# CMU-SAFARI/Genome-on-Diet

Hardware: AMD Instinct MI355X
Metric: mapped bases/sec (whole node), HiFi map-hifi k19w19 (higher is better)
Workload: dtype int16

## Files before the change

### genome-on-diet_amd/csrc/ksw_wave.hip.h

```cpp
#pragma once
#include <hip/hip_runtime.h>
#include <type_traits>
#include "ksw_common.h"
#include "ksw_wave_core.h"

template <int LANES> __device__ __forceinline__ u32 gdw_ror1(u32 v)
{
	if (LANES != 16) return (u32)__builtin_amdgcn_mov_dpp((int)v, 0x13C, 0xF, 0xF, true);
	return (u32)__builtin_amdgcn_mov_dpp((int)v, 0x121, 0xF, 0xF, true);
}

__device__ __forceinline__ u32 gdw_seam_byte(const uint8_t *query, int qlen, int j)
{
	if (j < 0 || j >= qlen) return 0u;
	const uintptr_t a = (uintptr_t)(query + j);
	typedef const __attribute__((address_space(4))) u32 *gdw_const_u32p;
	const u32 wd = *(gdw_const_u32p)(a & ~(uintptr_t)3);
	return (wd >> (8 * (a & 3))) & 0xffu;
}

__device__ __forceinline__ void gdw_band_uniform(int r, int qlen, int tlen, int w, int &st0, int &en0)
{
	r = __builtin_amdgcn_readfirstlane(r);
	int a = r - qlen + 1, b = (r - w + 1) >> 1, c = (r + w) >> 1, t1 = tlen - 1, st, en;
// ... 3 lines not shown
}

__device__ __forceinline__ const uint8_t *gdw_uniform_ptr(const uint8_t *p, int src_lane)
{
	const uintptr_t a = (uintptr_t)p;
	const u32 lo = (u32)__builtin_amdgcn_readlane((int)(u32)a, src_lane), hi = (u32)__builtin_amdgcn_readlane((int)(u32)(a >> 32), src_lane);
	return (const uint8_t *)((uintptr_t)hi << 32 | lo);
}
__device__ __forceinline__ int64_t gdw_uniform_i64(int64_t v)
{
	const u32 lo = (u32)__builtin_amdgcn_readfirstlane((int)(u32)(uint64_t)v), hi = (u32)__builtin_amdgcn_readfirstlane((int)(u32)((uint64_t)v >> 32));
	return (int64_t)((uint64_t)hi << 32 | lo);
}

#if __has_builtin(__builtin_amdgcn_writelane)
#define GDW_WRITELANE __builtin_amdgcn_writelane
#else
extern "C" __device__ int gdw_llvm_writelane_i32(int, int, int) __asm("llvm.amdgcn.writelane.i32");
#define GDW_WRITELANE gdw_llvm_writelane_i32
#endif
__device__ __forceinline__ u32 gdw_writelane_u(u32 value_uniform, int lane_uniform, u32 old)
{
	return (u32)GDW_WRITELANE(__builtin_amdgcn_readfirstlane((int)value_uniform), __builtin_amdgcn_readfirstlane(lane_uniform), (int)old);
}

__device__ __forceinline__ int gdw_narrow_rows(const WaveK &K, const uint8_t *query_u , const uint8_t *query, int qlen,
                                               const uint8_t *target, int tlen, int w, int lane, __amdgpu_buffer_rsrc_t bt_rsrc)
{
	typedef u32 gdw_u32x2 __attribute__((ext_vector_type(2)));
	const int rend = qlen + tlen - 2, mlast = (tlen - 1) >> 4, sl = (tlen - 1) & 15;
	WaveHalf H;
	gdw_load_half(H, K, lane >> 1, lane & 1, 0, query, qlen, target, tlen);
	bool any_tn = __builtin_amdgcn_ballot_w64(H.tn != 0) != 0;
	int prev_st_ = 0, prev_st0 = -1, prev_up = -1, prev_en0 = -1, have_f = 0, Rf = 0;
	auto store_row = [&](const int r, const u32 out[2]) __attribute__((always_inline)) {
		const gdw_u32x2 d = {out[0], out[1]};
		__builtin_amdgcn_raw_buffer_store_b64(d, bt_rsrc, lane * 8, r * 512, 0);
	};
	auto dp_row = [&](const int r, auto steady_tag) __attribute__((always_inline)) {
		constexpr bool STEADY = decltype(steady_tag)::value;
		WaveRow W;
		W.r = r;
		gdw_band_uniform(r, qlen, tlen, w, W.st0, W.en0);
		W.st_ = W.st0 >> 4, W.en_ = W.en0 >> 4;
		W.up = W.st0 + (((W.en0 - W.st0 + 16) >> 4) << 4);
		const int advanced = W.st_ > prev_st_;
		W.use_array = advanced;
		W.v1key = STEADY ? K.key_open : (W.st_ == 0 ? gdw_edge_key(K, r) : K.key_open);
		W.set_tr = STEADY ? 0 : (W.en0 | 15) >= r;
		W.ukey = STEADY ? 0 : gdw_edge_key(K, r);
		const u32 pX = gdw_ror1<64>(H.X[3]), pV = gdw_ror1<64>(H.V[3]), pX2 = gdw_ror1<64>(H.X2[3]), pQ = gdw_ror1<64>(H.Qc[1]);
		if (STEADY || r > 0) gdw_shift_query_half(H, pQ, H.blk == prev_st_ && H.half == 0, gdw_seam_byte(query_u, qlen, r - (prev_st_ << 4)));
		if (advanced) {
			if (H.blk < W.st_) gdw_load_half(H, K, H.blk + 32, H.half, r, query, qlen, target, tlen);
			any_tn = __builtin_amdgcn_ballot_w64(H.tn != 0) != 0;
		}
		if (!STEADY && W.set_tr) gdw_reset_tr_half(H, K, W);
		if (W.st0 != prev_st0 || W.up != prev_up || advanced) gdw_make_sel_half(H, W.st0, W.up);
		gdw_update_scores_half(H, K, any_tn);
		if (H.blk <= W.en_) {
			u32 out[2];
			gdw_compute_half<true>(H, K, W, pX, pV, pX2, out);
			store_row(r, out);
		}
		if (!STEADY && r == 0) H.R = gdw_lo(H.V[0]) - K.B1 - K.qe8;
		else H.R += gdw_lo(H.V[0]) - K.B1;
		if ((STEADY || r > 0) && W.en0 != prev_en0 && (W.en0 & 7) == 0) {
			const int hh = (int)gdw_ror1<64>((u32)gdw_track_handoff_half(H));
			if (H.blk == W.en_ && H.half == ((W.en0 >> 3) & 1)) H.R = hh + gdw_lo(H.U[0]);
		}
		if (!STEADY && W.en0 == tlen - 1) {
			if (H.blk == mlast && H.half == (sl >> 3)) {
				if (!have_f) Rf = gdw_track_to_slot_half(H, sl & 7);
				else Rf += gdw_cell_half(H.V, sl & 7) - K.B1;
			}
			have_f = 1;
		}
		prev_st_ = W.st_, prev_st0 = W.st0, prev_up = W.up, prev_en0 = W.en0;
	};
	const int nblkA = (w - 1 + 16) >> 4, nblkB = (w + 16) >> 4;
	u32 m_lowest = 0;
	const int step_mask = nblkA == nblkB ? 15 : 0;
	int m_full = 0;
	auto pair_row = [&](const int r, const int m, auto a_tag) __attribute__((always_inline)) {
		constexpr bool ROW_A = decltype(a_tag)::value;
		WaveRow W;
		W.r = r, W.st0 = m, W.en0 = ROW_A ? m + w - 1 : m + w;
		W.st_ = m >> 4, W.en_ = W.en0 >> 4;
		W.up = m + ((ROW_A ? nblkA : nblkB) << 4);
		const int advanced = ROW_A && (m & 15) == 0;
		const int pst_ = (m - (ROW_A ? 1 : 0)) >> 4;
		W.use_array = advanced, W.v1key = K.key_open, W.set_tr = 0, W.ukey = 0;
		const u32 pX = gdw_ror1<64>(H.X[3]), pV = gdw_ror1<64>(H.V[3]), pX2 = gdw_ror1<64>(H.X2[3]), pQ = gdw_ror1<64>(H.Qc[1]);
		gdw_shift_query_half_m(H, pQ, m_lowest, gdw_seam_byte(query_u, qlen, r - (pst_ << 4)));
		if (advanced) {
			if (H.blk < W.st_) gdw_load_half(H, K, H.blk + 32, H.half, r, query, qlen, target, tlen);
			any_tn = __builtin_amdgcn_ballot_w64(H.tn != 0) != 0;
		}
		if (ROW_A ? (m & step_mask) == 0 || m == m_full : nblkA != nblkB) {
			gdw_make_sel_half(H, W.st0, W.up);
			m_lowest = (H.blk == W.st_ && H.half == 0) ? ~0u : 0u;
		} else if (ROW_A) {
			const GdwSelStep S = gdw_sel_step_half(m, w);
#pragma unroll
			for (int k = 0; k < 2; ++k)
#pragma unroll
				for (int g = 0; g < 2; ++g) H.SEL[g] = gdw_writelane_u(S.sel[k][g], S.lane[k], H.SEL[g]);
		}
		W.m_first_valid = 1, W.m_first_h = m_lowest;
		gdw_update_scores_half(H, K, any_tn);
		if (H.blk <= W.en_) {
			u32 out[2];
			gdw_compute_half<true>(H, K, W, pX, pV, pX2, out);
			store_row(r, out);
		}
		H.R += gdw_lo(H.V[0]);
		if (!ROW_A && (W.en0 & 7) == 0) {
			const int hh = (int)gdw_ror1<64>((u32)gdw_track_handoff_half(H));
			if (H.blk == W.en_ && H.half == ((W.en0 >> 3) & 1)) H.R = hh + gdw_lo(H.U[0]);
		}
	};
	{
		int rA, rS;
		gdw_steady_rows(qlen, tlen, w, rA, rS);
		const int t1_ = tlen - 1, rB0 = 2 * t1_ - w, rB = rB0 > t1_ ? rB0 : t1_;
		int r = 0;
		for (; r <= rend && r < rA; ++r) dp_row(r, std::false_type());
		if (r == rA && rS > rA) {
			int m = (rA - w + 1) >> 1;
			m_full = m;
			m_lowest = (H.blk == prev_st_ && H.half == 0) ? ~0u : 0u;
			for (; r < rS; r += 2, ++m) {
				pair_row(r, m, std::true_type());
				pair_row(r + 1, m, std::false_type());
			}
			H.R -= (rS - rA) * K.B1;
			--m;
			prev_st_ = m >> 4, prev_st0 = m, prev_up = m + (nblkB << 4), prev_en0 = m + w;
		}
		for (; r <= rend && r < rB; ++r) dp_row(r, std::true_type());
		for (; r <= rend; ++r) dp_row(r, std::false_type());
	}
	return __builtin_amdgcn_readlane(Rf, (2 * mlast + (sl >> 3)) & 63);
}

__device__ __forceinline__ int gdw_quarter_rows(const WaveK &K, const uint8_t *query_u , const uint8_t *query, int qlen,
                                               const uint8_t *target, int tlen, int w, int lane, __amdgpu_buffer_rsrc_t bt_rsrc)
{
	const int rend = qlen + tlen - 2, mlast = (tlen - 1) >> 4, sl = (tlen - 1) & 15;
	WaveQuarter H;
	gdw_load_quarter(H, K, lane >> 2, lane & 3, 0, query, qlen, target, tlen);
	bool any_tn = __builtin_amdgcn_ballot_w64(H.tn != 0) != 0;
	int prev_st_ = 0, prev_st0 = -1, prev_up = -1, prev_en0 = -1, have_f = 0, Rf = 0;
	auto store_row = [&](const int r, const u32 out) __attribute__((always_inline)) {
		__builtin_amdgcn_raw_buffer_store_b32(out, bt_rsrc, lane * 4, r * 256, 0);
	};
	auto dp_row = [&](const int r, auto steady_tag) __attribute__((always_inline)) {
		constexpr bool STEADY = decltype(steady_tag)::value;
		WaveRow W;
		W.r = r;
		gdw_band_uniform(r, qlen, tlen, w, W.st0, W.en0);
		W.st_ = W.st0 >> 4, W.en_ = W.en0 >> 4;
		W.up = W.st0 + (((W.en0 - W.st0 + 16) >> 4) << 4);
		const int advanced = W.st_ > prev_st_;
		W.use_array = advanced;
		W.v1key = STEADY ? K.key_open : (W.st_ == 0 ? gdw_edge_key(K, r) : K.key_open);
		W.set_tr = STEADY ? 0 : (W.en0 | 15) >= r;
		W.ukey = STEADY ? 0 : gdw_edge_key(K, r);
		const u32 pX = gdw_ror1<64>(H.X[1]), pV = gdw_ror1<64>(H.V[1]), pX2 = gdw_ror1<64>(H.X2[1]), pQ = gdw_ror1<64>(H.Qc);
		if (STEADY || r > 0) gdw_shift_query_quarter(H, pQ, H.blk == prev_st_ && H.quarter == 0, gdw_seam_byte(query_u, qlen, r - (prev_st_ << 4)));
		if (advanced) {
			if (H.blk < W.st_) gdw_load_quarter(H, K, H.blk + 16, H.quarter, r, query, qlen, target, tlen);
			any_tn = __builtin_amdgcn_ballot_w64(H.tn != 0) != 0;
		}
		if (!STEADY && W.set_tr) gdw_reset_tr_quarter(H, K, W);
		if (W.st0 != prev_st0 || W.up != prev_up || advanced) gdw_make_sel_quarter(H, W.st0, W.up);
		gdw_update_scores_quarter(H, K, any_tn);
		if (H.blk <= W.en_) {
			u32 out;
			gdw_compute_quarter(H, K, W, pX, pV, pX2, out);
			store_row(r, out);
		}
		if (!STEADY && r == 0) H.R = gdw_lo(H.V[0]) - K.B1 - K.qe8;
		else H.R += gdw_lo(H.V[0]) - K.B1;
		if ((STEADY || r > 0) && W.en0 != prev_en0 && (W.en0 & 3) == 0) {
			const int hh = (int)gdw_ror1<64>((u32)gdw_track_handoff_quarter(H));
			if (H.blk == W.en_ && H.quarter == ((W.en0 >> 2) & 3)) H.R = hh + gdw_lo(H.U[0]);
		}
		if (!STEADY && W.en0 == tlen - 1) {
			if (H.blk == mlast && H.quarter == (sl >> 2)) {
				if (!have_f) Rf = gdw_track_to_slot_quarter(H, sl & 3);
				else Rf += gdw_cell_quarter(H.V, sl & 3) - K.B1;
			}
			have_f = 1;
		}
		prev_st_ = W.st_, prev_st0 = W.st0, prev_up = W.up, prev_en0 = W.en0;
	};
	const int nblkA = (w - 1 + 16) >> 4, nblkB = (w + 16) >> 4;
	u32 m_lowest = 0;
	const int step_mask = nblkA == nblkB ? 15 : 0;
	int m_full = 0;
	auto pair_row = [&](const int r, const int m, auto a_tag) __attribute__((always_inline)) {
		constexpr bool ROW_A = decltype(a_tag)::value;
		WaveRow W;
		W.r = r, W.st0 = m, W.en0 = ROW_A ? m + w - 1 : m + w;
		W.st_ = m >> 4, W.en_ = W.en0 >> 4;
		W.up = m + ((ROW_A ? nblkA : nblkB) << 4);
		const int advanced = ROW_A && (m & 15) == 0;
		const int pst_ = (m - (ROW_A ? 1 : 0)) >> 4;
		W.use_array = advanced, W.v1key = K.key_open, W.set_tr = 0, W.ukey = 0;
		const u32 pX = gdw_ror1<64>(H.X[1]), pV = gdw_ror1<64>(H.V[1]), pX2 = gdw_ror1<64>(H.X2[1]), pQ = gdw_ror1<64>(H.Qc);
		gdw_shift_query_quarter_m(H, pQ, m_lowest, gdw_seam_byte(query_u, qlen, r - (pst_ << 4)));
		if (advanced) {
			if (H.blk < W.st_) gdw_load_quarter(H, K, H.blk + 16, H.quarter, r, query, qlen, target, tlen);
			any_tn = __builtin_amdgcn_ballot_w64(H.tn != 0) != 0;
		}
		if (ROW_A ? (m & step_mask) == 0 || m == m_full : nblkA != nblkB) {
			gdw_make_sel_quarter(H, W.st0, W.up);
			m_lowest = (H.blk == W.st_ && H.quarter == 0) ? ~0u : 0u;
		} else if (ROW_A) {
			const GdwSelStep S = gdw_sel_step_quarter(m, w);
			H.SEL = gdw_writelane_u(S.sel[0][0], S.lane[0], H.SEL);
			H.SEL = gdw_writelane_u(S.sel[1][0], S.lane[1], H.SEL);
		}
		W.m_first_valid = 1, W.m_first_h = m_lowest;
		gdw_update_scores_quarter(H, K, any_tn);
		if (H.blk <= W.en_) {
			u32 out;
			gdw_compute_quarter(H, K, W, pX, pV, pX2, out);
			store_row(r, out);
		}
		H.R += gdw_lo(H.V[0]);
		if (!ROW_A && (W.en0 & 3) == 0) {
			const int hh = (int)gdw_ror1<64>((u32)gdw_track_handoff_quarter(H));
			if (H.blk == W.en_ && H.quarter == ((W.en0 >> 2) & 3)) H.R = hh + gdw_lo(H.U[0]);
		}
	};
	{
		int rA, rS;
		gdw_steady_rows(qlen, tlen, w, rA, rS);
		const int t1_ = tlen - 1, rB0 = 2 * t1_ - w, rB = rB0 > t1_ ? rB0 : t1_;
		int r = 0;
		for (; r <= rend && r < rA; ++r) dp_row(r, std::false_type());
		if (r == rA && rS > rA) {
			int m = (rA - w + 1) >> 1;
			m_full = m;
			m_lowest = (H.blk == prev_st_ && H.quarter == 0) ? ~0u : 0u;
			for (; r < rS; r += 2, ++m) {
				pair_row(r, m, std::true_type());
				pair_row(r + 1, m, std::false_type());
			}
			H.R -= (rS - rA) * K.B1;
			--m;
			prev_st_ = m >> 4, prev_st0 = m, prev_up = m + (nblkB << 4), prev_en0 = m + w;
		}
		for (; r <= rend && r < rB; ++r) dp_row(r, std::true_type());
		for (; r <= rend; ++r) dp_row(r, std::false_type());
	}
	return __builtin_amdgcn_readlane(Rf, (4 * mlast + (sl >> 2)) & 63);
}

#define GD_CLOCK_SLOTS 16384
__device__ unsigned long long gd_clock_stamps[GD_CLOCK_SLOTS * 4];
template <int LANES, int TAG = 0, bool DUAL = true>
__global__ __launch_bounds__(256) __attribute__((amdgpu_waves_per_eu(LANES == 64 ? 5 : 4)))
void ksw_extd2_wave_kernel(const KswTask *__restrict__ tasks,
                                                             const int32_t *__restrict__ task_ids, int n_slots,
                                                             const uint8_t *__restrict__ qseq,
                                                             const uint8_t *__restrict__ tseq,
                                                             uint8_t *__restrict__ bt, int32_t *__restrict__ status,
                                                             int32_t *__restrict__ score_out, WaveK K,
                                                             int32_t *__restrict__ n_cigar, uint32_t *__restrict__ cigar,
                                                             GdNarrowArg NA, uint32_t *__restrict__ narrow_cnt)
{
	constexpr int NG = 64 / LANES;
	const int lane = threadIdx.x & 63;
	const bool spare = lane >= NG * LANES;
	const int sub = spare ? lane - NG * LANES : lane % LANES, row = spare ? 0 : lane / LANES;
	const int slot = __builtin_amdgcn_readfirstlane((int)(blockIdx.x * (blockDim.x >> 6) + (threadIdx.x >> 6)));
	if (slot >= n_slots) return;
	int tid, live = 1;
	if (LANES == 64) {
		if (DUAL && NA.drain > 0 && slot >= __builtin_amdgcn_readfirstlane((int)narrow_cnt[GD_CNT_PENDING])) return;
		tid = __builtin_amdgcn_readfirstlane(task_ids[slot]);
		if (__builtin_amdgcn_readfirstlane(status[tid]) != GD_ST_PENDING) return;
	} else {
		tid = task_ids[NG * slot + row];
		const int tid0 = __builtin_amdgcn_readfirstlane(tid);
		if (tid < 0 || spare) tid = tid0, live = 0;
		else if (status[tid] != GD_ST_PENDING) live = 0;
		if (!__builtin_amdgcn_ballot_w64(live)) return;
	}
	const KswTask *Tp = tasks + tid;
	if (LANES == 64 && lane == 0) gd_clock_stamps[(tid & (GD_CLOCK_SLOTS - 1)) * 4] = __builtin_amdgcn_s_memtime(), gd_clock_stamps[(tid & (GD_CLOCK_SLOTS - 1)) * 4 + 1] = __builtin_amdgcn_s_memrealtime();
	const int qlen = __builtin_amdgcn_readfirstlane(Tp->qlen), tlen = __builtin_amdgcn_readfirstlane(Tp->tlen);
	int w = __builtin_amdgcn_readfirstlane(Tp->w);
	if (w < 0) w = tlen > qlen ? tlen : qlen;
	const uint8_t *query = qseq + Tp->qoff, *target = tseq + Tp->toff;
	uint8_t *p = bt + Tp->bt_off + (size_t)sub * 16;
	const int rend = qlen + tlen - 2, mlast = (tlen - 1) >> 4, sl = (tlen - 1) & 15;
	const uint8_t *qg[NG];
#pragma unroll
	for (int g = 0; g < NG; ++g) qg[g] = gdw_uniform_ptr(query, g * LANES);

	typedef u32 gdw_u32x4 __attribute__((ext_vector_type(4)));
	int64_t bt_base = LANES == 64 ? gdw_uniform_i64(Tp->bt_off) : 0;
	__amdgpu_buffer_rsrc_t bt_rsrc = __builtin_amdgcn_make_buffer_rsrc(bt + bt_base, 0, (int)0xffffffffu, 0x00020000);
	auto store_row = [&](const int r, const u32 out[4]) __attribute__((always_inline)) {
		if (LANES == 64) {
			const gdw_u32x4 d = {out[0], out[1], out[2], out[3]};
			__builtin_amdgcn_raw_buffer_store_b128(d, bt_rsrc, lane * 16, r * (LANES * 16), 0);
		} else if (live) *reinterpret_cast<uint4 *>(p + (size_t)r * (LANES * 16)) = make_uint4(out[0], out[1], out[2], out[3]);
	};
	if constexpr (LANES == 64 && DUAL) {
		const int mode = NA.w > 0 && cigar != nullptr ? __builtin_amdgcn_readfirstlane(Tp->pad) : GD_NARROW_NO;
		bool claim = NA.drain > 0;
		if (mode != GD_NARROW_NO) {
			int s8 = 0, wn = 0, stride = 0;
			const int wq = __builtin_amdgcn_readfirstlane(gd_quarter_rung(mode, qlen, tlen, w, NA.wq));
			if (wq > 0) {
				s8 = gdw_quarter_rows(K, qg[0], query, qlen, target, tlen, wq, lane, bt_rsrc);
				GdNarrowArg NQ = NA;
				NQ.w = wq;
				const bool own = wq == w, ok = own || gd_band_certified(NQ, qlen, tlen, s8 >> 3);
				if (!own && lane == 0) {
					atomicAdd(narrow_cnt + 2, 1u);
					if (ok) atomicAdd(narrow_cnt + 3, 1u);
				}
				if (ok) wn = wq, stride = 256;
			}
// ... 900 lines not shown
```

### genome-on-diet_amd/csrc/ksw_wave_core.h

```cpp
#pragma once
#include <stddef.h>
#include <stdint.h>
#include "ksw_common.h"

#if defined(__HIPCC__)
#define GDW_HD __host__ __device__ __forceinline__
#else
#define GDW_HD static inline
#endif

typedef uint32_t u32;

#if defined(__HIP_DEVICE_COMPILE__)
typedef short gdw_v2s __attribute__((ext_vector_type(2)));
GDW_HD gdw_v2s gdw_as_v(u32 a) { return __builtin_bit_cast(gdw_v2s, a); }
GDW_HD u32 gdw_as_u(gdw_v2s a) { return __builtin_bit_cast(u32, a); }
GDW_HD u32 pk_add(u32 a, u32 b) { return gdw_as_u(gdw_as_v(a) + gdw_as_v(b)); }
GDW_HD u32 pk_sub(u32 a, u32 b) { return gdw_as_u(gdw_as_v(a) - gdw_as_v(b)); }
GDW_HD u32 pk_max(u32 a, u32 b) { return gdw_as_u(__builtin_elementwise_max(gdw_as_v(a), gdw_as_v(b))); }
GDW_HD u32 pk_min(u32 a, u32 b) { return gdw_as_u(__builtin_elementwise_min(gdw_as_v(a), gdw_as_v(b))); }
GDW_HD u32 gdw_perm(u32 s0, u32 s1, u32 sel) { return __builtin_amdgcn_perm(s0, s1, sel); }
GDW_HD u32 gdw_alignbit(u32 hi, u32 lo, u32 sh) { return __builtin_amdgcn_alignbit(hi, lo, sh); }
GDW_HD u32 gdw_alignbyte(u32 hi, u32 lo, u32 sh) { return __builtin_amdgcn_alignbyte(hi, lo, sh); }
#else
GDW_HD u32 pk_add(u32 a, u32 b) { return ((a + b) & 0xffffu) | ((((a >> 16) + (b >> 16)) & 0xffffu) << 16); }
GDW_HD u32 pk_sub(u32 a, u32 b) { return ((a - b) & 0xffffu) | ((((a >> 16) - (b >> 16)) & 0xffffu) << 16); }
GDW_HD u32 pk_max(u32 a, u32 b)
{
	int16_t al = (int16_t)a, bl = (int16_t)b, ah = (int16_t)(a >> 16), bh = (int16_t)(b >> 16);
	return (u32)(uint16_t)(al > bl ? al : bl) | (u32)(uint16_t)(ah > bh ? ah : bh) << 16;
}
GDW_HD u32 pk_min(u32 a, u32 b)
{
	int16_t al = (int16_t)a, bl = (int16_t)b, ah = (int16_t)(a >> 16), bh = (int16_t)(b >> 16);
	return (u32)(uint16_t)(al < bl ? al : bl) | (u32)(uint16_t)(ah < bh ? ah : bh) << 16;
}
GDW_HD u32 gdw_perm(u32 s0, u32 s1, u32 sel)
{
	uint64_t src = (uint64_t)s0 << 32 | s1;
	u32 out = 0;
	for (int i = 0; i < 4; ++i) {
		u32 s = (sel >> (8 * i)) & 0xff, b;
		if (s <= 7) b = (u32)(src >> (8 * s)) & 0xff;
		else if (s == 12) b = 0;
		else if (s >= 13) b = 0xff;
		else b = ((src >> (16 * (s - 8) + 15)) & 1) ? 0xff : 0;
		out |= b << (8 * i);
	}
	return out;
}
GDW_HD u32 gdw_alignbit(u32 hi, u32 lo, u32 sh) { return (u32)((((uint64_t)hi << 32) | lo) >> (sh & 31)); }
GDW_HD u32 gdw_alignbyte(u32 hi, u32 lo, u32 sh) { return (u32)((((uint64_t)hi << 32) | lo) >> (8 * (sh & 3))); }
#endif
GDW_HD u32 gdw_bfi(u32 mask, u32 a, u32 b) { return (a & mask) | (b & ~mask); }
#if defined(__HIP_DEVICE_COMPILE__)
GDW_HD u32 gdw_bfi_u(u32 mask, u32 a, u32 b)
{
	u32 d;
	asm("v_bfi_b32 %0, %1, %2, %3" : "=v"(d) : "s"(mask), "v"(a), "v"(b));
	return d;
}
#else
GDW_HD u32 gdw_bfi_u(u32 mask, u32 a, u32 b) { return gdw_bfi(mask, a, b); }
#endif
GDW_HD u32 gdw_pack2(int v) { return ((u32)v & 0xffffu) | ((u32)v << 16); }
GDW_HD int gdw_lo(u32 a) { return (int)(int16_t)(a & 0xffffu); }
GDW_HD int gdw_hi(u32 a) { return (int)(int16_t)(a >> 16); }

struct WaveK {
	int32_t B1;
	u32 cx, cy, cx2, cy2;
	u32 c2;
	u32 uv0;
	u32 zmax;
	u32 te, te2;
	u32 lut_lo, lut_hi;
	u32 s0;
	int32_t key_open, key_e, key_ld, key_e2;
	int32_t long_thres;
	int32_t qe8;
};

static inline bool gdw_make_consts(const KswConst &C, WaveK &K)
{
	const int qe = C.q + C.e, qe2 = C.q2 + C.e2;
	K.B1 = 8 * (qe - 1);
	if (qe < 1) return false;
	K.cx = gdw_pack2(8 * -qe + 3 + K.B1), K.cy = gdw_pack2(8 * -qe + 2 + K.B1);
	const int B2 = 8 * (qe2 - 1);
	K.cx2 = gdw_pack2(8 * -qe2 + 1 + B2), K.cy2 = gdw_pack2(8 * -qe2 + B2);
	K.c2 = gdw_pack2(K.B1 - B2);
	K.uv0 = gdw_pack2(8 * -qe + K.B1);
	K.zmax = gdw_pack2(8 * C.sc_mch + 2 * K.B1);
	K.te = gdw_pack2(8 * (C.q - 1)), K.te2 = gdw_pack2(K.B1 - 8 * C.e2);
	const int km = 8 * C.sc_mch + 4 + 2 * K.B1, kx = 8 * C.sc_mis + 4 + 2 * K.B1, kn = 8 * C.sc_N + 4 + 2 * K.B1, k0 = 4 + 2 * K.B1;
	if (km < 0 || km > 255 || kx < 0 || kx > 255 || kn < 0 || kn > 255 || k0 > 255) return false;
	K.lut_lo = (u32)km | (u32)kx << 8 | (u32)kx << 16 | (u32)kx << 24;
	K.lut_hi = (u32)kn * 0x01010101u;
	K.s0 = (u32)k0 * 0x01010101u;
	K.key_open = 8 * -qe + K.B1, K.key_e = 8 * -C.e + K.B1, K.key_ld = 8 * C.long_diff + K.B1, K.key_e2 = 8 * -C.e2 + K.B1;
	K.long_thres = C.long_thres;
	K.qe8 = 8 * qe;
	if (8 * 127 + 7 + 2 * K.B1 > 30000) return false;
	return true;
}

GDW_HD int gdw_edge_key(const WaveK &K, int r)
{
	return r == 0 ? K.key_open : r < K.long_thres ? K.key_e : r == K.long_thres ? K.key_ld : K.key_e2;
}

struct WaveLane {
	u32 U[8], V[8], X[8], Y[8], X2[8], Y2[8];
	u32 Sb[4];
	u32 Tb[4];
	u32 Qc[4];
	u32 SEL[4];
	u32 tn;
	int32_t blk;
	int32_t R;
};

GDW_HD u32 gdw_qbyte(const uint8_t *query, int qlen, int j) { return (j >= 0 && j < qlen) ? query[j] : 0u; }

GDW_HD void gdw_load_block(WaveLane &L, const WaveK &K, int m, int r, const uint8_t *query, int qlen,
                           const uint8_t *target, int tlen)
{
	L.blk = m;
	const int tb = m << 4;
#pragma unroll
	for (int k = 0; k < 8; ++k) L.U[k] = K.uv0, L.V[k] = K.uv0, L.X[k] = K.cx, L.Y[k] = K.cy, L.X2[k] = K.cx2, L.Y2[k] = K.cy2;
#pragma unroll
	for (int g = 0; g < 4; ++g) {
		u32 tw = 0, qw = 0;
#pragma unroll
		for (int b = 0; b < 4; ++b) {
			const int t = tb + 4 * g + b;
			tw |= (t < tlen ? (u32)target[t] : 0u) << (8 * b);
			qw |= gdw_qbyte(query, qlen, r - t) << (8 * b);
		}
		L.Tb[g] = tw, L.Qc[g] = qw, L.Sb[g] = K.s0, L.SEL[g] = 0x03020100u;
	}
	L.tn = (L.Tb[0] | L.Tb[1] | L.Tb[2] | L.Tb[3]) & 0x04040404u;
	L.R = 0;
}

GDW_HD void gdw_fresh_block(WaveLane &L, const WaveK &K, int blk, int rq, const uint8_t *query, int qlen, const uint8_t *target, int tlen)
{
	const int tb = blk * 16;
	L.blk = blk;
#pragma unroll
	for (int k = 0; k < 8; ++k) L.U[k] = K.uv0, L.V[k] = K.uv0, L.X[k] = K.cx, L.Y[k] = K.cy, L.X2[k] = K.cx2, L.Y2[k] = K.cy2;
#pragma unroll
	for (int g = 0; g < 4; ++g) {
		u32 tw = 0, qw = 0;
#pragma unroll
		for (int b = 0; b < 4; ++b) {
			const int t = tb + 4 * g + b;
			tw |= (t >= 0 && t < tlen ? (u32)target[t] : 0u) << (8 * b);
			qw |= gdw_qbyte(query, qlen, rq - t) << (8 * b);
		}
		L.Tb[g] = tw, L.Qc[g] = qw, L.Sb[g] = K.s0, L.SEL[g] = 0x03020100u;
	}
	L.tn = (L.Tb[0] | L.Tb[1] | L.Tb[2] | L.Tb[3]) & 0x04040404u;
	L.R = 0;
}

struct WaveRow {
	int r, st0, en0, st_, en_, up;
	int use_array;
	int v1key;
	int set_tr;
	int ukey;
	int m_first_valid = 0;
	u32 m_first = 0, m_first_h = 0;
};

GDW_HD void gdw_make_sel(WaveLane &L, int st0, int up)
{
	const int tb = L.blk << 4;
	int lo = st0 - tb, hi = up - tb;
	lo = lo < 0 ? 0 : lo > 16 ? 16 : lo;
	hi = hi < 0 ? 0 : hi > 16 ? 16 : hi;
	const u32 bm = hi > lo ? (((1u << (hi - lo)) - 1u) << lo) : 0u;
#pragma unroll
	for (int g = 0; g < 4; ++g) {
		const u32 n = (bm >> (4 * g)) & 15u;
		const u32 spread = (n * 0x00204081u) & 0x01010101u;
		L.SEL[g] = 0x03020100u + (spread << 2);
	}
}

GDW_HD void gdw_sel_uniform(int d0, u32 lo[4], u32 hi[4])
{
	const uint64_t C = 0x0404040404040404ull;
	const uint64_t f0 = d0 < 8 ? C << (8 * d0) : 0ull, f1 = d0 < 8 ? C : C << (8 * (d0 - 8));
	lo[0] = 0x03020100u + (u32)f0, lo[1] = 0x03020100u + (u32)(f0 >> 32), lo[2] = 0x03020100u + (u32)f1, lo[3] = 0x03020100u + (u32)(f1 >> 32);
#pragma unroll
	for (int g = 0; g < 4; ++g) hi[g] = 0x0a080604u - lo[g];
}
#if defined(__HIP_DEVICE_COMPILE__)
GDW_HD u32 gdw_bfi_s(u32 mask, u32 a_uniform, u32 b)
{
	u32 d;
	asm("v_bfi_b32 %0, %1, %2, %3" : "=v"(d) : "v"(mask), "s"(a_uniform), "v"(b));
	return d;
}
// ... 185 lines not shown
		if (e0 != tlen - 1 || s0 > 16 * mlast) return false;
	}
	return true;
}

static inline bool gd_wave_scoring_ok(const KswConst &C)
{
	WaveK K;
	if (!gdw_make_consts(C, K)) return false;
	const int mis = C.sc_mis < 0 ? -C.sc_mis : C.sc_mis, n = C.sc_N < 0 ? -C.sc_N : C.sc_N;
	return C.sc_mch > 0 && C.sc_mch + 2 * (C.q2 + C.e2) + (mis > n ? mis : n) + (C.q + C.e) <= 120;
}

static inline bool gd_wave_supported(int qlen, int tlen, int w, int lanes)
{
	return qlen + tlen < (1 << 21) && gd_wave_geometry_ok(qlen, tlen, w, lanes);
}

#define GD_CK_ROWS 480
#define GD_CK_REGS 136
static inline __host__ __device__ size_t gd_ck_bytes(int qlen, int tlen, int )
{
	const size_t rows = (size_t)qlen + tlen - 1, n_ck = (rows + GD_CK_ROWS - 1) / GD_CK_ROWS;
	return n_ck * (size_t)GD_CK_REGS * 64 * 4 + (size_t)GD_CK_ROWS * 1024;
}

struct WaveHalf {
	u32 U[4], V[4], X[4], Y[4], X2[4], Y2[4];
	u32 Sb[2], Tb[2], Qc[2], SEL[2];
	u32 tn;
	int32_t blk, half;
	int32_t R;
};

GDW_HD void gdw_load_half(WaveHalf &H, const WaveK &K, int m, int half, int r, const uint8_t *query, int qlen, const uint8_t *target, int tlen)
{
	H.blk = m, H.half = half;
	const int tb = (m << 4) + (half << 3);
#pragma unroll
	for (int k = 0; k < 4; ++k) H.U[k] = K.uv0, H.V[k] = K.uv0, H.X[k] = K.cx, H.Y[k] = K.cy, H.X2[k] = K.cx2, H.Y2[k] = K.cy2;
#pragma unroll
	for (int g = 0; g < 2; ++g) {
		u32 tw = 0, qw = 0;
#pragma unroll
		for (int b = 0; b < 4; ++b) {
			const int t = tb + 4 * g + b;
			tw |= (t < tlen ? (u32)target[t] : 0u) << (8 * b);
			qw |= gdw_qbyte(query, qlen, r - t) << (8 * b);
		}
		H.Tb[g] = tw, H.Qc[g] = qw, H.Sb[g] = K.s0, H.SEL[g] = 0x03020100u;
	}
	H.tn = (H.Tb[0] | H.Tb[1]) & 0x04040404u;
	H.R = 0;
}

GDW_HD u32 gdw_sel_from_range_half(int lo, int hi, int g)
{
	const u32 bm = hi > lo ? (((1u << (hi - lo)) - 1u) << lo) : 0u;
	const u32 n = (bm >> (4 * g)) & 15u;
	const u32 spread = (n * 0x00204081u) & 0x01010101u;
	return 0x03020100u + (spread << 2);
}
GDW_HD void gdw_make_sel_half(WaveHalf &H, int st0, int up)
{
	const int tb = (H.blk << 4) + (H.half << 3);
	int lo = st0 - tb, hi = up - tb;
	lo = lo < 0 ? 0 : lo > 8 ? 8 : lo;
	hi = hi < 0 ? 0 : hi > 8 ? 8 : hi;
#pragma unroll
	for (int g = 0; g < 2; ++g) H.SEL[g] = gdw_sel_from_range_half(lo, hi, g);
}

struct GdwSelStep {
	int lane[2];
	int word[2];
	u32 sel[2][2];
};
GDW_HD GdwSelStep gdw_sel_step_half(int m, int w)
{
	const int up = m + (((w + 15) >> 4) << 4), c = (m - 1) & 7;
	GdwSelStep S;
	S.lane[0] = ((m - 1) >> 3) & 63, S.lane[1] = ((up - 1) >> 3) & 63;
	S.word[0] = S.word[1] = c >> 2;
#pragma unroll
	for (int g = 0; g < 2; ++g) S.sel[0][g] = gdw_sel_from_range_half(c + 1, 8, g), S.sel[1][g] = gdw_sel_from_range_half(0, c + 1, g);
	return S;
}

GDW_HD void gdw_shift_query_m(WaveLane &L, u32 below, u32 m_lowest, u32 seam)
{
	const u32 in = gdw_bfi_s(m_lowest, seam << 24, below);
	L.Qc[3] = gdw_alignbyte(L.Qc[3], L.Qc[2], 3);
	L.Qc[2] = gdw_alignbyte(L.Qc[2], L.Qc[1], 3);
	L.Qc[1] = gdw_alignbyte(L.Qc[1], L.Qc[0], 3);
	L.Qc[0] = gdw_alignbyte(L.Qc[0], in, 3);
}

GDW_HD void gdw_shift_query_half(WaveHalf &H, u32 below, bool is_lowest, u32 seam)
{
	const u32 in = is_lowest ? (seam << 24) : below;
	H.Qc[1] = gdw_alignbyte(H.Qc[1], H.Qc[0], 3);
	H.Qc[0] = gdw_alignbyte(H.Qc[0], in, 3);
}

GDW_HD void gdw_shift_query_half_m(WaveHalf &H, u32 below, u32 m_lowest, u32 seam)
{
	const u32 in = gdw_bfi_s(m_lowest, seam << 24, below);
	H.Qc[1] = gdw_alignbyte(H.Qc[1], H.Qc[0], 3);
	H.Qc[0] = gdw_alignbyte(H.Qc[0], in, 3);
}

GDW_HD void gdw_update_scores_half(WaveHalf &H, const WaveK &K, bool any_tn)
{
#pragma unroll
	for (int g = 0; g < 2; ++g) {
		u32 x = H.Tb[g] ^ H.Qc[g];
		if (any_tn) x |= H.Tb[g] & ~(H.Qc[g] << 1) & 0x04040404u;
		H.Sb[g] = gdw_perm(gdw_perm(K.lut_hi, K.lut_lo, x), H.Sb[g], H.SEL[g]);
	}
}

GDW_HD void gdw_reset_tr_half(WaveHalf &H, const WaveK &K, const WaveRow &W)
{
	if (H.blk != (W.r >> 4) || H.half != ((W.r >> 3) & 1)) return;
	const int c = W.r & 7, k = c & 3;
	const u32 mask = (c & 4) ? 0xffff0000u : 0x0000ffffu;
	const u32 uk = gdw_pack2(W.ukey);
#pragma unroll
	for (int kk = 0; kk < 4; ++kk)
		if (kk == k) {
			H.U[kk] = gdw_bfi(mask, uk, H.U[kk]);
			H.Y[kk] = gdw_bfi(mask, K.cy, H.Y[kk]);
			H.Y2[kk] = gdw_bfi(mask, K.cy2, H.Y2[kk]);
		}
}

template <bool BT = false>
GDW_HD void gdw_compute_half(WaveHalf &H, const WaveK &K, const WaveRow &W, u32 pX, u32 pV, u32 pX2, u32 *bt = nullptr)
{
	if (!W.use_array) {
		const u32 first = W.m_first_valid ? W.m_first_h : ((H.blk == W.st_ && H.half == 0) ? ~0u : 0u);
		pX = gdw_bfi_s(first, K.cx, pX), pV = gdw_bfi_s(first, gdw_pack2(W.v1key), pV), pX2 = gdw_bfi_s(first, K.cx2, pX2);
	}
	const u32 inX = gdw_alignbit(H.X[3], pX, 16), inV = gdw_alignbit(H.V[3], pV, 16), inX2 = gdw_alignbit(H.X2[3], pX2, 16);
	u32 zk_hi = 0;
#pragma unroll
	for (int k = 3; k >= 0; --k) {
		const u32 xin = k ? H.X[k - 1] : inX, vin = k ? H.V[k - 1] : inV, x2in = k ? H.X2[k - 1] : inX2;
		const u32 sk = gdw_perm(H.Sb[1], H.Sb[0], 0x0c000c00u | (u32)k | (u32)(4 + k) << 16);
		const u32 a = pk_add(xin, vin), b = pk_add(H.Y[k], H.U[k]);
		const u32 a2 = pk_add(x2in, vin), b2 = pk_add(H.Y2[k], H.U[k]);
		const u32 zk = pk_max(pk_max(pk_max(sk, a), b), pk_add(pk_max(a2, b2), K.c2));
		const u32 z8 = pk_min(zk & 0xfff8fff8u, K.zmax);
		const u32 nV = pk_sub(z8, H.U[k]), nU = pk_sub(z8, vin);
		const u32 tE = pk_sub(z8, K.te), tE2 = pk_sub(z8, K.te2);
		H.X[k] = pk_max(pk_sub(a, tE), K.cx), H.Y[k] = pk_max(pk_sub(b, tE), K.cy);
		H.X2[k] = pk_max(pk_sub(a2, tE2), K.cx2), H.Y2[k] = pk_max(pk_sub(b2, tE2), K.cy2);
		H.U[k] = nU, H.V[k] = nV;
		if (BT) {
			if (k & 1) zk_hi = zk;
			else {
				const u32 mX = gdw_perm(H.X[k + 1], H.X[k], 0x0b090a08u), mY = gdw_perm(H.Y[k + 1], H.Y[k], 0x0b090a08u);
				const u32 mX2 = gdw_perm(H.X2[k + 1], H.X2[k], 0x0b090a08u), mY2 = gdw_perm(H.Y2[k + 1], H.Y2[k], 0x0b090a08u);
				const u32 f = gdw_bfi_u(0x80808080u, mX, gdw_bfi_u(0x40404040u, mY, gdw_bfi_u(0x20202020u, mX2, mY2)));
				bt[k >> 1] = gdw_bfi_u(0xf0f0f0f0u, f, gdw_perm(zk_hi, zk, 0x06020400u));
			}
		}
	}
}

GDW_HD u32 gdw_half_pick(u32 rj, u32 rj4, int h) { return h ? (rj >> 16) | (rj4 & 0xffff0000u) : (rj & 0xffffu) | (rj4 << 16); }
GDW_HD void gdw_half_from_lane(const WaveLane &L, int h, WaveHalf &H)
{
#pragma unroll
	for (int j = 0; j < 4; ++j) {
		H.U[j] = gdw_half_pick(L.U[j], L.U[j + 4], h), H.V[j] = gdw_half_pick(L.V[j], L.V[j + 4], h);
		H.X[j] = gdw_half_pick(L.X[j], L.X[j + 4], h), H.Y[j] = gdw_half_pick(L.Y[j], L.Y[j + 4], h);
		H.X2[j] = gdw_half_pick(L.X2[j], L.X2[j + 4], h), H.Y2[j] = gdw_half_pick(L.Y2[j], L.Y2[j + 4], h);
	}
#pragma unroll
	for (int g = 0; g < 2; ++g) {
		H.Sb[g] = h ? L.Sb[2 + g] : L.Sb[g], H.Tb[g] = h ? L.Tb[2 + g] : L.Tb[g];
		H.Qc[g] = h ? L.Qc[2 + g] : L.Qc[g], H.SEL[g] = h ? L.SEL[2 + g] : L.SEL[g];
	}
	H.tn = (H.Tb[0] | H.Tb[1]) & 0x04040404u;
	H.blk = L.blk, H.half = h, H.R = 0;
}
GDW_HD void gdw_fresh_half(WaveHalf &H, const WaveK &K, int blk, int half, int rq, const uint8_t *query, int qlen, const uint8_t *target, int tlen)
{
	const int tb = blk * 16 + half * 8;
	H.blk = blk, H.half = half;
#pragma unroll
	for (int k = 0; k < 4; ++k) H.U[k] = K.uv0, H.V[k] = K.uv0, H.X[k] = K.cx, H.Y[k] = K.cy, H.X2[k] = K.cx2, H.Y2[k] = K.cy2;
#pragma unroll
	for (int g = 0; g < 2; ++g) {
		u32 tw = 0, qw = 0;
#pragma unroll
		for (int b = 0; b < 4; ++b) {
			const int t = tb + 4 * g + b;
			tw |= (t >= 0 && t < tlen ? (u32)target[t] : 0u) << (8 * b);
			qw |= gdw_qbyte(query, qlen, rq - t) << (8 * b);
		}
// ... 81 lines not shown
GDW_HD int gd_gap_cost(const GdNarrowArg &A, int k)
{
	if (k <= 0) return 0;
	const int c1 = A.q + k * A.e, c2 = A.q2 + k * A.e2;
	return c1 < c2 ? c1 : c2;
}
GDW_HD bool gd_band_certified(const GdNarrowArg &A, int qlen, int tlen, int score)
{
	const int D = A.w, delta = tlen - qlen;
	if (delta > D || -delta > D) return false;
	bool ok = true;
	if (D - delta >= 0) {
		const int l1 = qlen - (D - delta), l2 = tlen - D;
		const int ub = A.a * (l1 < l2 ? l1 : l2) - gd_gap_cost(A, D) - gd_gap_cost(A, D - delta);
		ok = ok && score > ub;
	}
	if (D + delta >= 0) {
		const int l1 = qlen - D, l2 = tlen - (D + delta);
		const int ub = A.a * (l1 < l2 ? l1 : l2) - gd_gap_cost(A, D) - gd_gap_cost(A, D + delta);
		ok = ok && score > ub;
	}
	return ok;
}

enum : int32_t { GD_NARROW_NO = 0,
                 GD_NARROW_TRY = 1,
                 GD_NARROW_OWN = 2 };
static inline int32_t gd_narrow_mode(int qlen, int tlen, int w)
{
	if (w < 0) w = tlen > qlen ? tlen : qlen;
	if (w <= GD_W_NARROW) return gd_narrow_supported(qlen, tlen, w) ? GD_NARROW_OWN : GD_NARROW_NO;
	const int delta = tlen - qlen;
	if (delta > GD_W_NARROW || -delta > GD_W_NARROW) return GD_NARROW_NO;
	return gd_narrow_supported(qlen, tlen, GD_W_NARROW) ? GD_NARROW_TRY : GD_NARROW_NO;
}

#define GD_W_QUARTER 239
struct WaveQuarter {
	u32 U[2], V[2], X[2], Y[2], X2[2], Y2[2];
	u32 Sb, Tb, Qc, SEL;
	u32 tn;
	int32_t blk, quarter;
	int32_t R;
};

GDW_HD void gdw_load_quarter(WaveQuarter &H, const WaveK &K, int m, int quarter, int r, const uint8_t *query, int qlen, const uint8_t *target, int tlen)
{
	H.blk = m, H.quarter = quarter;
	const int tb = (m << 4) + (quarter << 2);
#pragma unroll
	for (int k = 0; k < 2; ++k) H.U[k] = K.uv0, H.V[k] = K.uv0, H.X[k] = K.cx, H.Y[k] = K.cy, H.X2[k] = K.cx2, H.Y2[k] = K.cy2;
	u32 tw = 0, qw = 0;
#pragma unroll
	for (int b = 0; b < 4; ++b) {
		const int t = tb + b;
		tw |= (t < tlen ? (u32)target[t] : 0u) << (8 * b);
		qw |= gdw_qbyte(query, qlen, r - t) << (8 * b);
	}
	H.Tb = tw, H.Qc = qw, H.Sb = K.s0, H.SEL = 0x03020100u;
	H.tn = H.Tb & 0x04040404u;
	H.R = 0;
}

GDW_HD u32 gdw_sel_from_range_quarter(int lo, int hi)
{
	const u32 n = hi > lo ? (((1u << (hi - lo)) - 1u) << lo) : 0u;
	const u32 spread = (n * 0x00204081u) & 0x01010101u;
	return 0x03020100u + (spread << 2);
}
GDW_HD void gdw_make_sel_quarter(WaveQuarter &H, int st0, int up)
{
	const int tb = (H.blk << 4) + (H.quarter << 2);
	int lo = st0 - tb, hi = up - tb;
	lo = lo < 0 ? 0 : lo > 4 ? 4 : lo;
	hi = hi < 0 ? 0 : hi > 4 ? 4 : hi;
	H.SEL = gdw_sel_from_range_quarter(lo, hi);
}
GDW_HD GdwSelStep gdw_sel_step_quarter(int m, int w)
{
	const int up = m + (((w + 15) >> 4) << 4), c = (m - 1) & 3;
	GdwSelStep S;
	S.lane[0] = ((m - 1) >> 2) & 63, S.lane[1] = ((up - 1) >> 2) & 63;
	S.word[0] = S.word[1] = 0;
	S.sel[0][0] = gdw_sel_from_range_quarter(c + 1, 4), S.sel[1][0] = gdw_sel_from_range_quarter(0, c + 1);
	S.sel[0][1] = S.sel[1][1] = 0;
	return S;
}

GDW_HD void gdw_shift_query_quarter(WaveQuarter &H, u32 below, bool is_lowest, u32 seam)
{
	const u32 in = is_lowest ? (seam << 24) : below;
	H.Qc = gdw_alignbyte(H.Qc, in, 3);
}
GDW_HD void gdw_shift_query_quarter_m(WaveQuarter &H, u32 below, u32 m_lowest, u32 seam)
{
	const u32 in = gdw_bfi_s(m_lowest, seam << 24, below);
	H.Qc = gdw_alignbyte(H.Qc, in, 3);
}

GDW_HD void gdw_update_scores_quarter(WaveQuarter &H, const WaveK &K, bool any_tn)
{
	u32 x = H.Tb ^ H.Qc;
	if (any_tn) x |= H.Tb & ~(H.Qc << 1) & 0x04040404u;
	H.Sb = gdw_perm(gdw_perm(K.lut_hi, K.lut_lo, x), H.Sb, H.SEL);
}

GDW_HD void gdw_reset_tr_quarter(WaveQuarter &H, const WaveK &K, const WaveRow &W)
{
	if (H.blk != (W.r >> 4) || H.quarter != ((W.r >> 2) & 3)) return;
	const int c = W.r & 3, k = c & 1;
	const u32 mask = (c & 2) ? 0xffff0000u : 0x0000ffffu;
	const u32 uk = gdw_pack2(W.ukey);
#pragma unroll
	for (int kk = 0; kk < 2; ++kk)
		if (kk == k) {
			H.U[kk] = gdw_bfi(mask, uk, H.U[kk]);
			H.Y[kk] = gdw_bfi(mask, K.cy, H.Y[kk]);
			H.Y2[kk] = gdw_bfi(mask, K.cy2, H.Y2[kk]);
		}
}

GDW_HD void gdw_compute_quarter(WaveQuarter &H, const WaveK &K, const WaveRow &W, u32 pX, u32 pV, u32 pX2, u32 &bt)
{
	if (!W.use_array) {
		const u32 first = W.m_first_valid ? W.m_first_h : ((H.blk == W.st_ && H.quarter == 0) ? ~0u : 0u);
		pX = gdw_bfi_s(first, K.cx, pX), pV = gdw_bfi_s(first, gdw_pack2(W.v1key), pV), pX2 = gdw_bfi_s(first, K.cx2, pX2);
	}
	const u32 inX = gdw_alignbit(H.X[1], pX, 16), inV = gdw_alignbit(H.V[1], pV, 16), inX2 = gdw_alignbit(H.X2[1], pX2, 16);
	u32 zk_hi = 0;
#pragma unroll
	for (int k = 1; k >= 0; --k) {
		const u32 xin = k ? H.X[0] : inX, vin = k ? H.V[0] : inV, x2in = k ? H.X2[0] : inX2;
		const u32 sk = gdw_perm(0u, H.Sb, 0x0c000c00u | (u32)k | (u32)(2 + k) << 16);
		const u32 a = pk_add(xin, vin), b = pk_add(H.Y[k], H.U[k]);
		const u32 a2 = pk_add(x2in, vin), b2 = pk_add(H.Y2[k], H.U[k]);
		const u32 zk = pk_max(pk_max(pk_max(sk, a), b), pk_add(pk_max(a2, b2), K.c2));
		const u32 z8 = pk_min(zk & 0xfff8fff8u, K.zmax);
		const u32 nV = pk_sub(z8, H.U[k]), nU = pk_sub(z8, vin);
		const u32 tE = pk_sub(z8, K.te), tE2 = pk_sub(z8, K.te2);
		H.X[k] = pk_max(pk_sub(a, tE), K.cx), H.Y[k] = pk_max(pk_sub(b, tE), K.cy);
		H.X2[k] = pk_max(pk_sub(a2, tE2), K.cx2), H.Y2[k] = pk_max(pk_sub(b2, tE2), K.cy2);
		H.U[k] = nU, H.V[k] = nV;
		if (k) zk_hi = zk;
		else {
			const u32 mX = gdw_perm(H.X[1], H.X[0], 0x0b090a08u), mY = gdw_perm(H.Y[1], H.Y[0], 0x0b090a08u);
			const u32 mX2 = gdw_perm(H.X2[1], H.X2[0], 0x0b090a08u), mY2 = gdw_perm(H.Y2[1], H.Y2[0], 0x0b090a08u);
			const u32 f = gdw_bfi_u(0x80808080u, mX, gdw_bfi_u(0x40404040u, mY, gdw_bfi_u(0x20202020u, mX2, mY2)));
			bt = gdw_bfi_u(0xf0f0f0f0u, f, gdw_perm(zk_hi, zk, 0x06020400u));
		}
	}
}

GDW_HD int gdw_sum4(const u32 A[2])
{
	const u32 s = pk_add(A[0], A[1]);
	return gdw_lo(s) + gdw_hi(s);
}
GDW_HD int gdw_track_handoff_quarter(const WaveQuarter &H) { return H.R + gdw_sum4(H.U) - gdw_lo(H.U[0]) - gdw_sum4(H.V); }
GDW_HD int gdw_cell_quarter(const u32 A[2], int slot)
{
	const u32 a0 = A[0], a1 = A[1];
	const u32 v = (slot & 1) ? a1 : a0;
	return (slot & 2) ? gdw_hi(v) : gdw_lo(v);
}
GDW_HD int gdw_track_to_slot_quarter(const WaveQuarter &H, int sl)
{
	int acc = H.R;
	for (int i = 0; i < sl; ++i) acc += gdw_cell_quarter(H.U, i + 1) - gdw_cell_quarter(H.V, i);
	return acc;
}

GDW_HD bool gd_quarter_supported(int qlen, int tlen, int w)
{
	return qlen + tlen < (1 << 21) && gd_wave_geometry_ok(qlen, tlen, w, 16);
}
static inline bool gd_quarter_supported_loop(int qlen, int tlen, int w)
{
	return qlen + tlen < (1 << 21) && gd_wave_geometry_ok_loop(qlen, tlen, w, 16);
}
static inline bool gd_quarter_rows_ok(int qlen, int tlen, int w)
{
	if (w < 0) w = tlen > qlen ? tlen : qlen;
	if (qlen < 1 || tlen < 1 || w < 1 || qlen + tlen >= (1 << 21)) return false;
	if (gd_ncol16(qlen, tlen, w) > 16) return false;
	int prev_en0 = -1, have_f = 0;
	for (int r = 0; r <= qlen + tlen - 2; ++r) {
		int st0, en0;
// ... 23 lines not shown
```

Before: 2.414 billion.

## Stream seam query bytes through 64-bit window, simplify sel-step and N-base scoring

Result: faster. 2.502 billion (median of 6 runs) (+3.6%).

```diff
diff --git a/genome-on-diet_amd/csrc/ksw_wave.hip.h b/genome-on-diet_amd/csrc/ksw_wave.hip.h
--- a/genome-on-diet_amd/csrc/ksw_wave.hip.h
+++ b/genome-on-diet_amd/csrc/ksw_wave.hip.h
@@ -109,6 +109,10 @@
 	u32 m_lowest = 0;
 	const int step_mask = nblkA == nblkB ? 15 : 0;
 	int m_full = 0;
+	GdwSeam SQ = {0, 0};
+	u32 lut_lo_v = K.lut_lo;
+	GDW_KEEP_BRANCH(lut_lo_v);
+	u32 any_tn_u = 0;
 	auto pair_row = [&](const int r, const int m, auto a_tag) __attribute__((always_inline)) {
 		constexpr bool ROW_A = decltype(a_tag)::value;
 		WaveRow W;
@@ -116,13 +120,14 @@
 		W.st_ = m >> 4, W.en_ = W.en0 >> 4;
 		W.up = m + ((ROW_A ? nblkA : nblkB) << 4);
 		const int advanced = ROW_A && (m & 15) == 0;
-		const int pst_ = (m - (ROW_A ? 1 : 0)) >> 4;
 		W.use_array = advanced, W.v1key = K.key_open, W.set_tr = 0, W.ukey = 0;
 		const u32 pX = gdw_ror1<64>(H.X[3]), pV = gdw_ror1<64>(H.V[3]), pX2 = gdw_ror1<64>(H.X2[3]), pQ = gdw_ror1<64>(H.Qc[1]);
-		gdw_shift_query_half_m(H, pQ, m_lowest, gdw_seam_byte(query_u, qlen, r - (pst_ << 4)));
+		if (!ROW_A && (m & 15) == 0) gdw_seam_init(SQ, query_u, qlen, r, m);
+		gdw_shift_query_half_m(H, pQ, m_lowest, gdw_seam_next(SQ, query_u, qlen, r, m - (ROW_A ? 1 : 0)));
 		if (advanced) {
 			if (H.blk < W.st_) gdw_load_half(H, K, H.blk + 32, H.half, r, query, qlen, target, tlen);
-			any_tn = __builtin_amdgcn_ballot_w64(H.tn != 0) != 0;
+			const uint64_t bn = __builtin_amdgcn_ballot_w64(H.tn != 0);
+			any_tn = bn != 0, any_tn_u = (u32)bn | (u32)(bn >> 32);
 		}
 		if (ROW_A ? (m & step_mask) == 0 || m == m_full : nblkA != nblkB) {
 			gdw_make_sel_half(H, W.st0, W.up);
@@ -135,7 +140,7 @@
 				for (int g = 0; g < 2; ++g) H.SEL[g] = gdw_writelane_u(S.sel[k][g], S.lane[k], H.SEL[g]);
 		}
 		W.m_first_valid = 1, W.m_first_h = m_lowest;
-		gdw_update_scores_half(H, K, any_tn);
+		gdw_update_scores_half_n(H, K, any_tn_u, lut_lo_v);
 		if (H.blk <= W.en_) {
 			u32 out[2];
 			gdw_compute_half<true>(H, K, W, pX, pV, pX2, out);
@@ -157,6 +162,8 @@
 			int m = (rA - w + 1) >> 1;
 			m_full = m;
 			m_lowest = (H.blk == prev_st_ && H.half == 0) ? ~0u : 0u;
+			gdw_seam_init(SQ, query_u, qlen, r, m - 1);
+			any_tn_u = any_tn ? 1u : 0u;
 			for (; r < rS; r += 2, ++m) {
 				pair_row(r, m, std::true_type());
 				pair_row(r + 1, m, std::false_type());
@@ -227,6 +234,10 @@
 	u32 m_lowest = 0;
 	const int step_mask = nblkA == nblkB ? 15 : 0;
 	int m_full = 0;
+	GdwSeam SQ = {0, 0};
+	u32 lut_lo_v = K.lut_lo;
+	GDW_KEEP_BRANCH(lut_lo_v);
+	u32 any_tn_u = 0;
 	auto pair_row = [&](const int r, const int m, auto a_tag) __attribute__((always_inline)) {
 		constexpr bool ROW_A = decltype(a_tag)::value;
 		WaveRow W;
@@ -234,13 +245,14 @@
 		W.st_ = m >> 4, W.en_ = W.en0 >> 4;
 		W.up = m + ((ROW_A ? nblkA : nblkB) << 4);
 		const int advanced = ROW_A && (m & 15) == 0;
-		const int pst_ = (m - (ROW_A ? 1 : 0)) >> 4;
 		W.use_array = advanced, W.v1key = K.key_open, W.set_tr = 0, W.ukey = 0;
 		const u32 pX = gdw_ror1<64>(H.X[1]), pV = gdw_ror1<64>(H.V[1]), pX2 = gdw_ror1<64>(H.X2[1]), pQ = gdw_ror1<64>(H.Qc);
-		gdw_shift_query_quarter_m(H, pQ, m_lowest, gdw_seam_byte(query_u, qlen, r - (pst_ << 4)));
+		if (!ROW_A && (m & 15) == 0) gdw_seam_init(SQ, query_u, qlen, r, m);
+		gdw_shift_query_quarter_m(H, pQ, m_lowest, gdw_seam_next(SQ, query_u, qlen, r, m - (ROW_A ? 1 : 0)));
 		if (advanced) {
 			if (H.blk < W.st_) gdw_load_quarter(H, K, H.blk + 16, H.quarter, r, query, qlen, target, tlen);
-			any_tn = __builtin_amdgcn_ballot_w64(H.tn != 0) != 0;
+			const uint64_t bn = __builtin_amdgcn_ballot_w64(H.tn != 0);
+			any_tn = bn != 0, any_tn_u = (u32)bn | (u32)(bn >> 32);
 		}
 		if (ROW_A ? (m & step_mask) == 0 || m == m_full : nblkA != nblkB) {
 			gdw_make_sel_quarter(H, W.st0, W.up);
@@ -251,7 +263,7 @@
 			H.SEL = gdw_writelane_u(S.sel[1][0], S.lane[1], H.SEL);
 		}
 		W.m_first_valid = 1, W.m_first_h = m_lowest;
-		gdw_update_scores_quarter(H, K, any_tn);
+		gdw_update_scores_quarter_n(H, K, any_tn_u, lut_lo_v);
 		if (H.blk <= W.en_) {
 			u32 out;
 			gdw_compute_quarter(H, K, W, pX, pV, pX2, out);
@@ -273,6 +285,8 @@
 			int m = (rA - w + 1) >> 1;
 			m_full = m;
 			m_lowest = (H.blk == prev_st_ && H.quarter == 0) ? ~0u : 0u;
+			gdw_seam_init(SQ, query_u, qlen, r, m - 1);
+			any_tn_u = any_tn ? 1u : 0u;
 			for (; r < rS; r += 2, ++m) {
 				pair_row(r, m, std::true_type());
 				pair_row(r + 1, m, std::false_type());
diff --git a/genome-on-diet_amd/csrc/ksw_wave_core.h b/genome-on-diet_amd/csrc/ksw_wave_core.h
--- a/genome-on-diet_amd/csrc/ksw_wave_core.h
+++ b/genome-on-diet_amd/csrc/ksw_wave_core.h
@@ -62,6 +62,13 @@
 }
 #else
 GDW_HD u32 gdw_bfi_u(u32 mask, u32 a, u32 b) { return gdw_bfi(mask, a, b); }
+#endif
+#if defined(__HIP_DEVICE_COMPILE__)
+#define GDW_KEEP_BRANCH(v) asm volatile("" : "+v"(v))
+#define GDW_RARE_S(s) asm volatile("" : "+s"(s))
+#else
+#define GDW_KEEP_BRANCH(v) ((void)0)
+#define GDW_RARE_S(s) ((void)0)
 #endif
 GDW_HD u32 gdw_pack2(int v) { return ((u32)v & 0xffffu) | ((u32)v << 16); }
 GDW_HD int gdw_lo(u32 a) { return (int)(int16_t)(a & 0xffffu); }
@@ -123,6 +130,72 @@
 
 GDW_HD u32 gdw_qbyte(const uint8_t *query, int qlen, int j) { return (j >= 0 && j < qlen) ? query[j] : 0u; }
 
+#if defined(__HIP_DEVICE_COMPILE__)
+GDW_HD u32 gdw_seam_load(const uint8_t *p )
+{
+	typedef const __attribute__((address_space(4))) u32 *gdw_const_u32p;
+	return *(gdw_const_u32p)(uintptr_t)p;
+}
+GDW_HD uint64_t gdw_seam_load2(const uint8_t *p )
+{
+	typedef const __attribute__((address_space(4))) uint64_t *gdw_const_u64p;
+	return *(gdw_const_u64p)(uintptr_t)p;
+}
+#define GDW_SEAM_ORDER(w) asm volatile("" : "+s"(w) : : "memory")
+#else
+#ifndef GDW_SEAM_LOAD_HOOK
+#define GDW_SEAM_LOAD_HOOK(p) ((void)0)
+#endif
+GDW_HD u32 gdw_seam_load(const uint8_t *p)
+{
+	GDW_SEAM_LOAD_HOOK(p);
+	return (u32)p[0] | (u32)p[1] << 8 | (u32)p[2] << 16 | (u32)p[3] << 24;
+}
+GDW_HD uint64_t gdw_seam_load2(const uint8_t *p) { return (uint64_t)gdw_seam_load(p + 4) << 32 | gdw_seam_load(p); }
+#define GDW_SEAM_ORDER(w) ((void)0)
+#endif
+struct GdwSeam {
+	uint64_t win;
+	uint64_t nxt;
+};
+GDW_HD void gdw_seam_fetch(GdwSeam &S, const uint8_t *query, int qlen, int jb)
+{
+	if (jb + 4 < qlen) S.nxt = gdw_seam_load2(query + jb);
+	else if (jb < qlen) S.nxt = gdw_seam_load(query + jb);
+}
+GDW_HD uint64_t gdw_seam_inside(int qlen, int jb)
+{
+	int n = qlen - jb;
+	n = n < 0 ? 0 : n > 8 ? 8 : n;
+	return ~((~0ull << (4 * n)) << (4 * n));
+}
+GDW_HD int gdw_seam_pos(const uint8_t *query, int r) { return (int)(((u32)(uintptr_t)query + (u32)r) & 7u); }
+GDW_HD void gdw_seam_init(GdwSeam &S, const uint8_t *query, int qlen, int r, int mb)
+{
+	GDW_RARE_S(r);
+	GDW_RARE_S(mb);
+	const int pos = gdw_seam_pos(query, r);
+	const int jb = r - ((mb >> 4) << 4) - pos - (pos == 0 ? 8 : 0);
+	S.nxt = 0;
+	gdw_seam_fetch(S, query, qlen, jb);
+	S.win = S.nxt & gdw_seam_inside(qlen, jb);
+	gdw_seam_fetch(S, query, qlen, jb + 8);
+}
+GDW_HD u32 gdw_seam_next(GdwSeam &S, const uint8_t *query, int qlen, int r, int mb)
+{
+	const int pos = gdw_seam_pos(query, r);
+	if (pos == 0) {
+		GDW_RARE_S(r);
+		GDW_RARE_S(mb);
+		const int j = r - ((mb >> 4) << 4);
+		uint64_t w = S.nxt & gdw_seam_inside(qlen, j);
+		GDW_SEAM_ORDER(w);
+		S.win = w;
+		gdw_seam_fetch(S, query, qlen, j + 8);
+	}
+	return (u32)(S.win >> (8 * pos)) & 0xffu;
+}
+
 GDW_HD void gdw_load_block(WaveLane &L, const WaveK &K, int m, int r, const uint8_t *query, int qlen,
                            const uint8_t *target, int tlen)
 {
@@ -474,8 +547,9 @@
 	GdwSelStep S;
 	S.lane[0] = ((m - 1) >> 3) & 63, S.lane[1] = ((up - 1) >> 3) & 63;
 	S.word[0] = S.word[1] = c >> 2;
-#pragma unroll
-	for (int g = 0; g < 2; ++g) S.sel[0][g] = gdw_sel_from_range_half(c + 1, 8, g), S.sel[1][g] = gdw_sel_from_range_half(0, c + 1, g);
+	const uint64_t t = (0x0404040404040404ull << (8 * c)) << 8;
+#pragma unroll
+	for (int g = 0; g < 2; ++g) S.sel[0][g] = 0x03020100u + (u32)(t >> (32 * g)), S.sel[1][g] = 0x07060504u - (u32)(t >> (32 * g));
 	return S;
 }
 
@@ -510,6 +584,18 @@
 		if (any_tn) x |= H.Tb[g] & ~(H.Qc[g] << 1) & 0x04040404u;
 		H.Sb[g] = gdw_perm(gdw_perm(K.lut_hi, K.lut_lo, x), H.Sb[g], H.SEL[g]);
 	}
+}
+
+GDW_HD void gdw_update_scores_half_n(WaveHalf &H, const WaveK &K, u32 any_tn , u32 lut_lo )
+{
+	u32 x[2] = {H.Tb[0] ^ H.Qc[0], H.Tb[1] ^ H.Qc[1]};
+	if (any_tn != 0) {
+		u32 n0 = H.Tb[0] & ~(H.Qc[0] << 1) & 0x04040404u, n1 = H.Tb[1] & ~(H.Qc[1] << 1) & 0x04040404u;
+		GDW_KEEP_BRANCH(n0);
+		x[0] |= n0, x[1] |= n1;
+	}
+#pragma unroll
+	for (int g = 0; g < 2; ++g) H.Sb[g] = gdw_perm(gdw_perm(K.lut_hi, lut_lo, x[g]), H.Sb[g], H.SEL[g]);
 }
 
 GDW_HD void gdw_reset_tr_half(WaveHalf &H, const WaveK &K, const WaveRow &W)
@@ -757,7 +843,8 @@
 	GdwSelStep S;
 	S.lane[0] = ((m - 1) >> 2) & 63, S.lane[1] = ((up - 1) >> 2) & 63;
 	S.word[0] = S.word[1] = 0;
-	S.sel[0][0] = gdw_sel_from_range_quarter(c + 1, 4), S.sel[1][0] = gdw_sel_from_range_quarter(0, c + 1);
+	const u32 t = (u32)(0x0404040400ull << (8 * c));
+	S.sel[0][0] = 0x03020100u + t, S.sel[1][0] = 0x07060504u - t;
 	S.sel[0][1] = S.sel[1][1] = 0;
 	return S;
 }
@@ -778,6 +865,17 @@
 	u32 x = H.Tb ^ H.Qc;
 	if (any_tn) x |= H.Tb & ~(H.Qc << 1) & 0x04040404u;
 	H.Sb = gdw_perm(gdw_perm(K.lut_hi, K.lut_lo, x), H.Sb, H.SEL);
+}
+
+GDW_HD void gdw_update_scores_quarter_n(WaveQuarter &H, const WaveK &K, u32 any_tn , u32 lut_lo )
+{
+	u32 x = H.Tb ^ H.Qc;
+	if (any_tn != 0) {
+		u32 n = H.tn & ~(H.Qc << 1);
+		GDW_KEEP_BRANCH(n);
+		x |= n;
+	}
+	H.Sb = gdw_perm(gdw_perm(K.lut_hi, lut_lo, x), H.Sb, H.SEL);
 }
 
 GDW_HD void gdw_reset_tr_quarter(WaveQuarter &H, const WaveK &K, const WaveRow &W)
```
